# jacobwilliams/lbfgsb

Hardware: NVIDIA B200
Metric: lbfgsb_iterations_per_s (higher is better)
Workload: dtype f64

## Files before the change

### include/lbfgsb_b200.h

```cpp
#ifndef LBFGSB_B200_H
#define LBFGSB_B200_H

#include <stdint.h>

#ifdef __cplusplus
extern "C" {
#endif

#define LBFGSB_B200_MMAX 20

typedef struct lbfgsb_dev lbfgsb_dev_t;

int lbfgsb_b200_version(void);
const char* lbfgsb_b200_last_error(void);

void lbfgsb_setulb_f64(const int32_t* n, const int32_t* m, double* x, const double* l, const double* u,
                       const int32_t* nbd, double* f, double* g, const double* factr, const double* pgtol,
                       double* wa, int32_t* iwa, char* task, const int32_t* iprint, char* csave,
                       int32_t* lsave, int32_t* isave, double* dsave, const char* itfile, int32_t itfile_len);
void lbfgsb_setulb_f32(const int32_t* n, const int32_t* m, float* x, const float* l, const float* u,
                       const int32_t* nbd, float* f, float* g, const float* factr, const float* pgtol,
                       float* wa, int32_t* iwa, char* task, const int32_t* iprint, char* csave,
                       int32_t* lsave, int32_t* isave, float* dsave, const char* itfile, int32_t itfile_len);
void lbfgsb_host_release(int32_t* isave);
// ... 87 lines not shown

typedef struct lbfgsb_batch lbfgsb_batch_t;
lbfgsb_batch_t* lbfgsb_batch_create(int32_t nprob, int64_t n, int32_t m, int32_t real_kind, void* cuda_stream);
void lbfgsb_batch_destroy(lbfgsb_batch_t* h);
void lbfgsb_batch_setulb_dev_f64(lbfgsb_batch_t* h, double* x_dev, const double* l_dev, const double* u_dev, const int32_t* nbd_dev,
                                 double* f_dev, double* g_dev, const double* factr, const double* pgtol, char* task, char* csave,
                                 int32_t* lsave, int32_t* isave, double* dsave);
void lbfgsb_batch_setulb_dev_f32(lbfgsb_batch_t* h, float* x_dev, const float* l_dev, const float* u_dev, const int32_t* nbd_dev,
                                 float* f_dev, float* g_dev, const float* factr, const float* pgtol, char* task, char* csave,
                                 int32_t* lsave, int32_t* isave, float* dsave);
int lbfgsb_batch_counts(lbfgsb_batch_t* h, int32_t* n_fg, int32_t* n_newx, int32_t* n_done);
void* lbfgsb_batch_stream(lbfgsb_batch_t* h);
void* lbfgsb_batch_fg_mask(lbfgsb_batch_t* h);
int lbfgsb_batch_get_iwhere(lbfgsb_batch_t* h, int32_t* iwhere_host);
int lbfgsb_problem_rosenbrock_batch_f64(int32_t nprob, int64_t n, const double* x_dev, double* g_dev, double* f_dev,
                                        const int32_t* mask_dev, void* cuda_stream);
int lbfgsb_problem_rosenbrock_batch_f32(int32_t nprob, int64_t n, const float* x_dev, float* g_dev, float* f_dev,
                                        const int32_t* mask_dev, void* cuda_stream);

int lbfgsb_test_projgr_f64(int64_t n, const double* l, const double* u, const int32_t* nbd, const double* x,
                           const double* g, double* sbgnrm_out);
int lbfgsb_test_sum_f64(int64_t n, const double* a, const double* b, double* out);
int lbfgsb_test_sum_f32(int64_t n, const float* a, const float* b, float* out);
int lbfgsb_test_sort_f64(int64_t n, const double* t_dev, int32_t* order_out_dev, double* sorted_out_dev);
int lbfgsb_test_host_heap_group_f64(int64_t nb, const double* t_host, double tk, int32_t* group_out, int64_t* group_count);
int lbfgsb_test_heap_order_f64(int64_t n, const double* t_dev, int32_t* order_out_dev);
int lbfgsb_test_formk_delta_f64(int64_t n, int32_t m, int32_t col, int32_t head, int64_t ldw, const double* ws_dev,
                                const double* wy_dev, const unsigned char* state_dev, double* out_host);
int lbfgsb_test_formk_delta_f32(int64_t n, int32_t m, int32_t col, int32_t head, int64_t ldw, const float* ws_dev,
                                const float* wy_dev, const unsigned char* state_dev, float* out_host);
int lbfgsb_test_dense_f64(int32_t op, int32_t m, int32_t col, double theta, double* a, double* b, double* c,
                          int32_t* info);
int lbfgsb_test_dcsrch_f64(double f, double g, double* stp, double stpmax, int32_t* task, int32_t* isave2,
                           double* dsave13);

#ifdef __cplusplus
}
#endif
#endif
```

### lbfgsb_b200/csrc/common.cuh

```cuda
#pragma once
#include <cuda_runtime.h>
#include <stdint.h>
#include <float.h>
#include <math.h>

#include "../../include/lbfgsb_b200_shape.h"

typedef long long i64;

#define LB_MMAX 20
#define LB_KMAX (6 * LB_MMAX + 8)
#define LB_IMAX 8

enum {
    TK_START = 0, TK_FG_START = 1, TK_FG_LNSRCH = 2, TK_NEW_X = 3, TK_CONV_PG = 4, TK_CONV_F = 5,
    TK_ABNORMAL = 6, TK_RESTART = 7, TK_STOP = 8,
    TK_ERR_N = 10, TK_ERR_M = 11, TK_ERR_FACTR = 12, TK_ERR_NBD = 13, TK_ERR_INFEAS = 14
};
enum { PAUSE_NONE = 0, PAUSE_CLASSIFY = 1, PAUSE_WALK = 2, PAUSE_GCP_FREEV = 3, PAUSE_DELTA = 4, PAUSE_BACKTRACK = 5, PAUSE_LSINIT = 6 };
enum {
    CS_START = 0, CS_FG = 1, CS_CONV = 2, CS_WARN_ROUND = 3, CS_WARN_XTOL = 4, CS_WARN_STPMAX = 5,
    CS_WARN_STPMIN = 6, CS_ERR_STP_LT_MIN = 10, CS_ERR_STP_GT_MAX = 11, CS_ERR_G_GE_0 = 12,
    CS_ERR_FTOL = 13, CS_ERR_GTOL = 14, CS_ERR_XTOL = 15, CS_ERR_STPMIN = 16, CS_ERR_STPMAX = 17,
    CS_BLANK = 99
};
__host__ __device__ inline bool cs_is_warn(int c) { return c >= CS_WARN_ROUND && c <= CS_WARN_STPMIN; }
__host__ __device__ inline bool cs_is_err(int c) { return c >= CS_ERR_STP_LT_MIN && c <= CS_ERR_STPMAX; }
// ... 9 lines not shown
    EV_LNSRCH_RESTART = 8,
    EV_SKIP = 9,
    EV_FORMT_FAIL = 10
};
#define LB_EVMAX 24

template <typename T> struct Real;
template <> struct Real<double> {
    static constexpr int VEC = LBFGSB_VEC_F64;
    static constexpr int UNROLL = LBFGSB_UNROLL_F64;
    typedef double2 vec_t;
    typedef int2 ivec_t;
    typedef unsigned long long key_t;
    __host__ __device__ static double eps() { return DBL_EPSILON; }
};
template <> struct Real<float> {
    static constexpr int VEC = LBFGSB_VEC_F32;
    static constexpr int UNROLL = LBFGSB_UNROLL_F32;
    typedef float2 vec_t;
    typedef int2 ivec_t;
    typedef unsigned int key_t;
    __host__ __device__ static float eps() { return FLT_EPSILON; }
};

template <typename T>
struct DevState {
    int go;
    int pause;
    int in_body;
    int restart;
    int need_walk;
    int cauchy_mode;
    int do_subspace, do_formk, do_delta, do_backtrack, do_update, do_step, do_restore;
    int fuse_uc;
    int classify_done;
    int lsinit_done;
    int spec_step;
    int step_done;
    int do_unstep;
    int lazy_gcp;
    int fuse_gf;
    int lazy_z;
    int p2p_timeout;
    int z_in_x;
    int save_z;
    int task, csave, info;
// ... 706 lines not shown
```

### lbfgsb_b200/csrc/engine.cu

```cuda
#include <cuda_runtime.h>
#include <dlfcn.h>
#include <stdarg.h>
#include <stdio.h>
#include <stdlib.h>
#include <string.h>

#include <mutex>
#include <string>
#include <unordered_set>
#include <vector>

#include "../../include/lbfgsb_b200.h"
#include "cauchy_walk.cuh"
#include "kernels_tma.cuh"
#include "cauchy_walk_dist.cuh"
#include "batch.cuh"
#include "host_print.h"
#include <algorithm>

static thread_local std::string g_last_error;
static void set_error(const char* fmt, ...) {
    char buf[512];
    va_list ap;
    va_start(ap, fmt);
// ... 68 lines not shown
    __syncthreads();
    if (threadIdx.x == 0) *flag_host = seq;
}

__global__ void __launch_bounds__(256) k_publish_g(const unsigned* src, unsigned* dst_host, int words, volatile unsigned long long* flag_host,
                                                   unsigned long long* counter) {
    for (int q = threadIdx.x; q < words; q += blockDim.x) dst_host[q] = src[q];
    __threadfence_system();
    __syncthreads();
    if (threadIdx.x == 0) { const unsigned long long v = *counter + 1; *counter = v; *flag_host = v; }
}

struct EngineBase {
    virtual ~EngineBase() {}
    int real_kind;
    lbprint::Ctx pr;
};

template <typename T>
struct Engine : EngineBase {
    i64 n = 0, n_global = 0, offset = 0;
    int m = 0, mt = 0;
    bool fused = false;
    cudaStream_t stream = 0;
    bool own_stream = false;
    Wk<T> w;
    WalkBuf<T> wb;
    DevState<T>* s_dev = nullptr;
    DevState<T>* s_host = nullptr;
    size_t header_bytes = 0;
    int* tile_counts = nullptr; i64* tile_offsets = nullptr; i64 ntiles = 0;
    int* rs_counts = nullptr;
    SortCtl* ctl_el = nullptr;
    SortCtl* ctl_host = nullptr;
    T* tmpAB = nullptr; T* tmpF = nullptr; unsigned long long* jmin = nullptr;
    T* fd_parts = nullptr; T* delta = nullptr; T* delta_all = nullptr; T* delta_sum = nullptr;
    std::vector<void*> allocs;
    int R = 1, rank = 0;
    ncclComm_t comm = nullptr;
    Red<T>* rec_local = nullptr; Red<T>* rec_all = nullptr;
    unsigned long long* samp_local = nullptr; unsigned long long* samp_all = nullptr; unsigned long long* spl_dev = nullptr;
    DwCtl* dctl = nullptr; i64* pos_all = nullptr; SortCtl* ctl_d = nullptr;
    RoundRec* rr_local = nullptr; RoundRec* rr_all = nullptr;
    WalkCarry<T>* carry_local = nullptr; WalkCarry<T>* carry_all = nullptr;
    struct DynBuf { void* p = nullptr; size_t cap = 0; };
    DynBuf dw_send, dw_recv, dw_k0, dw_k1, dw_v0, dw_v1;
// ... 68 lines not shown
        p2p = true;
        for (int q = 0; q < R; ++q) p2p = p2p && oks[q];
        return true;
    }

    template <typename P> bool dalloc(P** p, size_t bytes) {
        void* q = nullptr;
        if (bytes == 0) bytes = 16;
        cudaError_t e = cudaMalloc(&q, bytes);
        if (e != cudaSuccess) { set_error("cudaMalloc(%zu) failed: %s", bytes, cudaGetErrorString(e)); return false; }
        allocs.push_back(q);
        *p = (P*)q;
        return true;
    }

    bool init(i64 n_, i64 off_, i64 ng_, int m_, cudaStream_t st, ncclComm_t cm, int rank_, int world_) {
        n = n_; offset = off_; n_global = ng_; m = m_; R = world_; rank = rank_; comm = cm;
        real_kind = (int)sizeof(T);
        mt = (m <= 5) ? 5 : (m <= 10 ? 10 : 20);
        fused = (mt == 5 ? fused_passes_ok<T, 5>() : (mt == 10 ? fused_passes_ok<T, 10>() : fused_passes_ok<T, 20>()));
        if (const char* e = getenv("LBFGSB_B200_NO_FUSION")) { if (e[0] == '1') fused = false; }
        fast = fused;
        if (const char* e = getenv("LBFGSB_B200_NO_FAST")) { if (e[0] == '1') fast = false; }
        if (const char* e = getenv("LBFGSB_B200_NO_TIMERS")) { if (e[0] == '1') timers = false; }
        if (const char* e = getenv("LBFGSB_B200_NO_SMALL_ROUNDS")) { if (e[0] == '1') { small_rounds = false; small_sort = false; } }
        if (const char* e = getenv("LBFGSB_B200_NO_BP_HINT")) { if (e[0] == '1') { bp_hint_ok = false; walk_gf_ok = false; } }
        if (!(mt == 5 ? set_smem_attrs<5>() : (mt == 10 ? set_smem_attrs<10>() : set_smem_attrs<20>()))) return false;
        for (int q = 0; q < F_COUNT; ++q) { fam_ms[q] = 0; fam_calls[q] = 0; }
        if (st) stream = st;
        else { CK(cudaStreamCreateWithFlags(&stream, cudaStreamNonBlocking)); own_stream = true; }
        memset(&w, 0, sizeof w);
        w.n = n; w.m = m; w.off = offset;
        w.ldw = (n + 31) / 32 * 32;
        const size_t vb = (size_t)w.ldw * sizeof(T);
        if (!dalloc(&w.ws, vb * m) || !dalloc(&w.wy, vb * m)) return false;
        if (!dalloc(&w.z, vb) || !dalloc(&w.r, vb) || !dalloc(&w.d, vb) || !dalloc(&w.t, vb) || !dalloc(&w.xp, vb) || !dalloc(&w.gold, vb)) return false;
        if (!dalloc(&w.iwhere, (size_t)w.ldw * 4) || !dalloc(&w.state, (size_t)w.ldw)) return false;
        if (!dalloc(&w.part, sizeof(T) * LB_KMAX * LBFGSB_GRID) || !dalloc(&w.ipart, sizeof(i64) * LB_IMAX * LBFGSB_GRID)) return false;
        if (!dalloc(&w.part2, sizeof(T) * LB_KMAX * LBFGSB_GRID) || !dalloc(&w.ipart2, sizeof(i64) * LB_IMAX * LBFGSB_GRID)) return false;
        if (!dalloc(&s_dev, sizeof(DevState<T>))) return false;
        CK(cudaMemsetAsync(s_dev, 0, sizeof(DevState<T>), stream));
        {
            i64 lim = (i64)1 << 28;
            if (R > 1) lim = (i64)1 << 26;
            if (const char* e = getenv("LBFGSB_B200_TIE_LIMIT")) lim = atoll(e);
            CK(cudaMemcpyAsync(&s_dev->tie_limit, &lim, sizeof lim, cudaMemcpyHostToDevice, stream));
        }
        CK(cudaMemsetAsync(w.ws, 0, vb * m, stream));
        CK(cudaMemsetAsync(w.wy, 0, vb * m, stream));
        w.s = s_dev;
        CK(cudaHostAlloc((void**)&s_host, sizeof(DevState<T>) + 64, cudaHostAllocMapped));
        memset(s_host, 0, sizeof(DevState<T>) + 64);
        pub_flag = (volatile unsigned long long*)((char*)s_host + ((sizeof(DevState<T>) + 7) / 8) * 8);
        if (const char* e = getenv("LBFGSB_B200_SYNC")) { if (e[0] == 'm') publish = false; }
        CK(cudaMallocHost((void**)&ctl_host, sizeof(SortCtl)));
// ... 152 lines not shown
        return true;
    }
#define LG LBFGSB_GRID, LBFGSB_BLOCK, 0, stream
#define LS 1, LB_SCALAR_THREADS, 0, stream
#define MTCALL(kern, smemfn, ...)                                                                          \
    do {                                                                                                   \
        if (mt == 5) kern<T, 5><<<LBFGSB_GRID, LB_TMA_THREADS, smemfn<T, 5>(), stream>>>(__VA_ARGS__);        \
        else if (mt == 10) kern<T, 10><<<LBFGSB_GRID, LB_TMA_THREADS, smemfn<T, 10>(), stream>>>(__VA_ARGS__); \
        else kern<T, 20><<<LBFGSB_GRID, LB_TMA_THREADS, smemfn<T, 20>(), stream>>>(__VA_ARGS__);              \
    } while (0)

    template <int MT> void launch_update_classify() {
        if constexpr (fused_passes_ok<T, MT>()) k_update_classify<T, MT><<<LBFGSB_GRID, LB_TMA_THREADS, smem_update_classify<T, MT>(), stream>>>(w);
    }
    template <int MT> void launch_formk_cmprlb() {
        if constexpr (fused_passes_ok<T, MT>()) k_formk_cmprlb<T, MT, 0><<<LBFGSB_GRID, LB_TMA_THREADS, smem_formk_cmprlb<T, MT>(), stream>>>(w);
    }
    template <int MT> void launch_formk_cmprlb_gf() {
        if constexpr (fused_passes_ok<T, MT>()) k_formk_cmprlb<T, MT, 1><<<LBFGSB_GRID, LB_TMA_THREADS, smem_formk_cmprlb<T, MT>(), stream>>>(w);
    }
    template <int MT> void launch_formk_cmprlb_gf2() {
        if constexpr (fused_passes_ok<T, MT>()) k_formk_cmprlb<T, MT, 2><<<LBFGSB_GRID, LB_TMA_THREADS, smem_formk_cmprlb<T, MT>(), stream>>>(w);
    }
    template <int MT> void launch_subsm_lsinit() {
        if constexpr (fused_passes_ok<T, MT>()) k_subsm_lsinit<T, MT, 0><<<LBFGSB_GRID, LB_TMA_THREADS, smem_subsm<T, MT>(), stream>>>(w);
    }
    template <int MT> void launch_subsm_dir() {
        if constexpr (fused_passes_ok<T, MT>()) k_subsm_lsinit<T, MT, 1><<<LBFGSB_GRID, LB_TMA_THREADS, smem_subsm<T, MT>(), stream>>>(w);
    }
#define MTFUSED(fn) do { if (mt == 5) fn<5>(); else if (mt == 10) fn<10>(); else fn<20>(); } while (0)

    template <int MT> bool set_smem_attrs() {
        CK(cudaFuncSetAttribute(k_update<T, MT>, cudaFuncAttributeMaxDynamicSharedMemorySize, (int)smem_update<T, MT>()));
        CK(cudaFuncSetAttribute(k_cauchy_classify<T, MT>, cudaFuncAttributeMaxDynamicSharedMemorySize, (int)smem_classify<T, MT>()));
        CK(cudaFuncSetAttribute(k_formk_gram<T, MT>, cudaFuncAttributeMaxDynamicSharedMemorySize, (int)smem_formk<T, MT>()));
        CK(cudaFuncSetAttribute(k_cmprlb_wv<T, MT>, cudaFuncAttributeMaxDynamicSharedMemorySize, (int)smem_cmprlb<T, MT>()));
        CK(cudaFuncSetAttribute(k_subsm_step<T, MT>, cudaFuncAttributeMaxDynamicSharedMemorySize, (int)smem_subsm<T, MT>()));
        if constexpr (fused_passes_ok<T, MT>()) {
            CK(cudaFuncSetAttribute(k_update_classify<T, MT>, cudaFuncAttributeMaxDynamicSharedMemorySize, (int)smem_update_classify<T, MT>()));
            CK(cudaFuncSetAttribute(k_formk_cmprlb<T, MT, 0>, cudaFuncAttributeMaxDynamicSharedMemorySize, (int)smem_formk_cmprlb<T, MT>()));
            CK(cudaFuncSetAttribute(k_formk_cmprlb<T, MT, 1>, cudaFuncAttributeMaxDynamicSharedMemorySize, (int)smem_formk_cmprlb<T, MT>()));
            CK(cudaFuncSetAttribute(k_formk_cmprlb<T, MT, 2>, cudaFuncAttributeMaxDynamicSharedMemorySize, (int)smem_formk_cmprlb<T, MT>()));
            CK(cudaFuncSetAttribute(k_subsm_lsinit<T, MT, 0>, cudaFuncAttributeMaxDynamicSharedMemorySize, (int)smem_subsm<T, MT>()));
            CK(cudaFuncSetAttribute(k_subsm_lsinit<T, MT, 1>, cudaFuncAttributeMaxDynamicSharedMemorySize, (int)smem_subsm<T, MT>()));
        }
        return true;
    }

    static unsigned long long key_of(T t) {
        typename Real<T>::key_t k;
        memcpy(&k, &t, sizeof k);
        return (unsigned long long)k;
    }
    int run_round(const BpRange& rg, bool first = false) {
        begin(F_WALK_COMPACT);
        if (first) k_bp_count<T, true><<<LG>>>(w, rg, tile_counts);
        else k_bp_count<T, false><<<LG>>>(w, rg, tile_counts);
        k_walk_round_local<T><<<1, 1024, 0, stream>>>(w, tile_counts, tile_offsets, ntiles, wb.ctl, rr_local);
        end(F_WALK_COMPACT, 2);
        if (R > 1 && !allgather(rr_local, rr_all, sizeof(RoundRec))) return -1;
        k_walk_round_begin<T><<<1, 32, 0, stream>>>(w, R > 1 ? rr_all : rr_local, R, n_global); launches++;
        if (!sync_state()) return -1;
        if (s_host->walk_closed) return 1;
        if (s_host->walk_rcount > 0) {
            begin(F_WALK_COMPACT); k_bp_write<T><<<LG>>>(w, rg, tile_counts, tile_offsets, wb.k0, wb.v0); end(F_WALK_COMPACT);
            begin(F_WALK_SORT); enqueue_sort(wb.k0, wb.k1, wb.v0, wb.v1, wb.ctl, s_host->walk_lcount); end(F_WALK_SORT, 0);
            if (R > 1) { if (!round_scan_sharded()) return -1; }
// ... 413 lines not shown
                    if (!site(site_freev())) return false;
                    begin(F_SCALAR); s_freev<T><<<LS>>>(w, dist(), n_global, 1); end(F_SCALAR);
                }
            }
            if (from <= PAUSE_DELTA) {
                if (from == PAUSE_DELTA) phase(PH_SUBSPACE);
                begin(F_FORMK_DELTA);
                k_el_count<T><<<LG>>>(w, tile_counts);
                k_tile_scan<T><<<1, 1024, 0, stream>>>(w, 1, tile_counts, tile_offsets, ntiles, ctl_el);
                k_flag_write<T, 1><<<LG>>>(w, tile_counts, tile_offsets, wb.k0, wb.v0);
                k_formk_delta<T><<<fd_grid<T>(), 256, 0, stream>>>(w, wb.v0, ctl_el, fd_parts);
                k_formk_delta_final<T><<<(6 * LB_MMAX * LB_MMAX + 255) / 256, 256, 0, stream>>>(w, fd_parts, fd_grid<T>(), delta);
                end(F_FORMK_DELTA, 5);
                if (!site(site_formk(mt))) return false;
                if (R > 1) {
                    if (p2p) { delta_seq++; k_delta_push<T><<<1, 256, 0, stream>>>(w, delta, peers_delta, peers, R, rank, delta_seq); launches++; }
                    else if (!allgather(delta, delta_all, sizeof(T) * 6 * LB_MMAX * LB_MMAX)) return false;
                }
                begin(F_SCALAR); s_formk_dense<T><<<LS>>>(w, dist(), mt, R > 1 ? delta_all : delta, delta_sum); end(F_SCALAR);
                if (!fused) { begin(F_CMPRLB_WV); MTCALL(k_cmprlb_wv, smem_cmprlb, w); end(F_CMPRLB_WV); }
                if (!site(site_wv(mt))) return false;
                begin(F_SCALAR); s_subsm_dense<T><<<LS>>>(w, dist(), mt, fused ? 1 : 0); end(F_SCALAR);
                if (fused) { begin(F_SUBSM_LSINIT); MTFUSED(launch_subsm_lsinit); end(F_SUBSM_LSINIT); }
                else { begin(F_SUBSM_STEP); MTCALL(k_subsm_step, smem_subsm, w); end(F_SUBSM_STEP); }
                if (!site(site_subsm())) return false;
                begin(F_SCALAR); s_subsm_post<T><<<LS>>>(w, dist(), fused ? 1 : 0); end(F_SCALAR);
            }
            if (from <= PAUSE_BACKTRACK) {
                if (from == PAUSE_BACKTRACK) phase(PH_SUBSPACE);
                begin(F_BACKTRACK);
                if (fused) { MTFUSED(launch_subsm_dir); launches++; }
                k_bt_alpha<T><<<LG>>>(w);
                if (!site(site_bt())) return false;
                s_bt<T><<<LS>>>(w, dist(), offset);
                k_bt_apply<T><<<LG>>>(w);
                end(F_BACKTRACK, 3);
            }
            phase(PH_LNSRCH);
            begin(F_LS_INIT); k_ls_init<T><<<LG>>>(w); end(F_LS_INIT);
            if (!site(site_lsinit())) return false;
            begin(F_SCALAR); s_ls_init<T><<<LS>>>(w, dist()); end(F_SCALAR);
            begin(F_LS_STEP); k_ls_step<T><<<LG>>>(w); end(F_LS_STEP);
            phase(PH_END);
            if (!sync_state()) return false;
            if (s_host->do_step) x_changed = true;
            if (!s_host->restart) break;
            begin(F_SCALAR); s_restart_body<T><<<1, 32, 0, stream>>>(w); end(F_SCALAR);
// ... 855 lines not shown
        T av[VEC], bv[VEC];
        ldv<T>(a, base, n, av); ldv<T>(b, base, n, bv);
#pragma unroll
        for (int v = 0; v < VEC; ++v) if (base + v < n) acc[0] = acc[0] + av[v] * bv[v];
    }
    block_sum_store<T, 1>(acc, 1, sm, part);
}
template <typename T>
__global__ void k_test_sum_final(const T* part, T* out) {
    T s = final_sum_warp<T>(part);
    if (threadIdx.x == 0) out[0] = s;
}
template <typename T>
static int test_sum_impl(i64 n, const T* a, const T* b, T* out) {
    T* part = nullptr;
    if (cudaMalloc(&part, sizeof(T) * (LBFGSB_GRID + 1)) != cudaSuccess) return 1;
    k_test_sum<T><<<LBFGSB_GRID, LBFGSB_BLOCK>>>(n, a, b, part);
    k_test_sum_final<T><<<1, 32>>>(part, part + LBFGSB_GRID);
    cudaError_t e = cudaMemcpy(out, part + LBFGSB_GRID, sizeof(T), cudaMemcpyDeviceToHost);
    cudaFree(part);
    return e != cudaSuccess;
}

__global__ void k_test_dense(int op, int m, int col, double theta, double* a, double* b, double* c, int* info, DevState<double>* st) {
    if (blockIdx.x != 0 || threadIdx.x >= 32) return;
    int r = 0;
    if (op >= 10 && op <= 14) {
        if (op == 10) r = wdense::dpofa<double>(a, m, col);
        else if (op == 11) r = wdense::dtrsl<double>(a, m, col, b, 1);
        else if (op == 12) r = wdense::dtrsl<double>(a, m, col, b, 11);
        else if (op == 13) r = wdense::bmv<double>(m, a, b, col, c, c + 2 * m);
        else r = wdense::formt<double>(m, c, a, b, col, theta);
        if (threadIdx.x == 0) *info = r;
        return;
    }
    if (op == 15) {
        if (threadIdx.x == 0) {
            st->m = m; st->col = col; st->theta = theta; st->do_formk = 1; st->updatd = 0; st->do_delta = 0; st->iupdat = m + 1;
            st->restart = 0; st->in_body = 1; st->ev_n = 0;
            for (int q = 0; q < m * m; ++q) st->sy[q] = b[q];
        }
        __syncwarp();
        Red<double>* red = nullptr;
        w_formk_dense<double>(st, *red, m <= 5 ? 5 : (m <= 10 ? 10 : 20), (const double*)nullptr, c, a);
        if (threadIdx.x == 0) *info = st->restart ? 1 : 0;
        return;
// ... 538 lines not shown
int lbfgsb_problem_quadratic_f32(int64_t n, const float* x, float* g, float* f_out, void* st, int64_t off, uint64_t seed,
                                 float xl, float xr, void* scratch) {
    return quadratic_impl<float>(n, x, g, f_out, st, off, seed, xl, xr, scratch);
}

int lbfgsb_test_projgr_f64(int64_t n, const double* l, const double* u, const int32_t* nbd, const double* x, const double* g,
                           double* out) {
    Wk<double> w; memset(&w, 0, sizeof w);
    DevState<double>* s = nullptr; double* part = nullptr;
    if (cudaMalloc(&s, sizeof(DevState<double>)) || cudaMalloc(&part, sizeof(double) * (LBFGSB_GRID + 1))) return 1;
    int one = 1;
    cudaMemcpy(&s->go, &one, sizeof(int), cudaMemcpyHostToDevice);
    w.n = n; w.l = l; w.u = u; w.nbd = nbd; w.x = (double*)x; w.g = (double*)g; w.part = part; w.s = s;
    k_projgr<double><<<LBFGSB_GRID, LBFGSB_BLOCK>>>(w);
    std::vector<double> hp(LBFGSB_GRID);
    cudaError_t e = cudaMemcpy(hp.data(), part, sizeof(double) * LBFGSB_GRID, cudaMemcpyDeviceToHost);
    double r = 0; for (double v : hp) r = v > r ? v : r;
    *out = r;
    cudaFree(s); cudaFree(part);
    return e != cudaSuccess;
}
int lbfgsb_test_sum_f64(int64_t n, const double* a, const double* b, double* out) { return test_sum_impl<double>(n, a, b, out); }
int lbfgsb_test_sum_f32(int64_t n, const float* a, const float* b, float* out) { return test_sum_impl<float>(n, a, b, out); }

int lbfgsb_test_sort_f64(int64_t n, const double* t, int32_t* order_out, double* sorted_out) {
    typedef unsigned long long K;
    K *k0, *k1; int *v0, *v1, *cnt; SortCtl* ctl;
    if (cudaMalloc(&k0, 8 * n) || cudaMalloc(&k1, 8 * n) || cudaMalloc(&v0, 4 * n) || cudaMalloc(&v1, 4 * n) ||
        cudaMalloc(&cnt, 4 * 256 * LB_RS_GRID) || cudaMalloc(&ctl, sizeof(SortCtl))) return 1;
    cudaMemcpy(k0, t, 8 * n, cudaMemcpyDeviceToDevice);
    k_test_iota<K><<<256, 256>>>(v0, n);
    k_test_setctl<<<1, 32>>>(ctl, n);
    for (int pass = 0; pass < 8; ++pass) {
        k_rs_hist<K><<<LB_RS_GRID, 256>>>(k0, k1, ctl, pass * 8, cnt);
        k_rs_scan<<<1, 1024>>>(cnt, ctl, LB_RS_GRID);
        k_rs_scatter<K><<<LB_RS_GRID, 256>>>(k0, k1, v0, v1, ctl, pass * 8, cnt);
        k_rs_flip<<<1, 32>>>(ctl);
    }
    SortCtl hc;
    cudaMemcpy(&hc, ctl, sizeof hc, cudaMemcpyDeviceToHost);
    cudaMemcpy(order_out, hc.cur ? v1 : v0, 4 * n, cudaMemcpyDeviceToDevice);
    cudaError_t e = cudaMemcpy(sorted_out, hc.cur ? k1 : k0, 8 * n, cudaMemcpyDeviceToDevice);
    cudaFree(k0); cudaFree(k1); cudaFree(v0); cudaFree(v1); cudaFree(cnt); cudaFree(ctl);
    return e != cudaSuccess || cudaGetLastError() != cudaSuccess;
}
int lbfgsb_test_host_heap_group_f64(int64_t nb, const double* t_host, double tk, int32_t* group_out, int64_t* group_count) {
// ... 135 lines not shown
```

### lbfgsb_b200/csrc/kernels_stream.cuh

```cuda
#pragma once
#include "common.cuh"

template <typename T>
struct Wk {
    i64 n, ldw;
    i64 off;
    int m;
    T *ws, *wy;
    T *z, *r, *d, *t, *xp;
    T* gold;
    int* iwhere;
    unsigned char* state;
    T* part;
    i64* ipart;
    T* part2;
    i64* ipart2;
    DevState<T>* s;
    T* x; const T* l; const T* u; const int* nbd; T* g;
    int bp_hint;
};

#define LB_SLOT(part, k) ((part) + (i64)(k) * LBFGSB_GRID)
#define LB_INF(T) ((T)INFINITY)
#define LB_I64MAX 0x7fffffffffffffffLL

template <typename T>
__global__ void __launch_bounds__(LBFGSB_BLOCK) k_errclb(Wk<T> w) {
    constexpr int VEC = Real<T>::VEC;
    i64 k6 = -1, k7 = -1;
    LB_FOR_TILES(T, w.n, base) {
        T l[VEC], u[VEC]; int nb[VEC];
        ldv<T>(w.l, base, w.n, l); ldv<T>(w.u, base, w.n, u); ldvi<T>(w.nbd, base, w.n, nb);
#pragma unroll
        for (int v = 0; v < VEC; ++v) {
            i64 i = base + v;
            if (i < w.n) {
                if (nb[v] < 0 || nb[v] > 3) k6 = i;
                if (nb[v] == 2 && l[v] > u[v]) k7 = i;
            }
        }
    }
    i64 m6 = k6, m7 = k7;
// ... 342 lines not shown
```

### lbfgsb_b200/csrc/kernels_tma.cuh

```cuda
#pragma once
#include "kernels_stream.cuh"
#include "tma_pipe.cuh"

template <typename T, int MT> struct SubT { static constexpr int v = (sizeof(T) * MT <= 80) ? 256 : 128; };

template <typename T> struct SpecializeFullHistory { static constexpr bool value = sizeof(T) == 4; };
template <bool B> struct BoolC { static constexpr bool value = B; };

#define LB_DYN_STAGES(dyn) (dyn)

template <typename T>
__device__ __forceinline__ void pipe_add_w(PipeSrc* ps, const Wk<T>& w, int head0, int count, unsigned slot) {
    int pj = head0;
    for (int j = 0; j < count; ++j) {
        pipe_add(ps, w.wy + (i64)pj * w.ldw, (int)sizeof(T), slot);
        pipe_add(ps, w.ws + (i64)pj * w.ldw, (int)sizeof(T), slot);
        pj = (pj + 1 == w.m) ? 0 : pj + 1;
    }
}

template <typename T, int MT>
__global__ void __launch_bounds__(LB_TMA_THREADS, 1) k_update(Wk<T> w) {
    constexpr int VEC = Real<T>::VEC;
    constexpr int SUBT = SubT<T, MT>::v;
// ... 291 lines not shown
                }
            }
        }
#pragma unroll
        for (int j = 0; j < MT; ++j) {
            if (j < col) {
                T wy[VEC], wsv[VEC];
                lds_real<T>(sb, OW + (2 * j) * G::REAL_SLOT, lt, wy);
                lds_real<T>(sb, OW + (2 * j + 1) * G::REAL_SLOT, lt, wsv);
#pragma unroll
                for (int v = 0; v < VEC; ++v)
                    if (fr[v]) {
                        acc[j] = acc[j] + wy[v] * r[v];
                        acc[MT + j] = acc[MT + j] + wsv[v] * r[v];
                    }
            }
        }
        stv<T>(w.r, base, n, r);
    });
    block_sum_store<T, 2 * MT>(acc, 2 * MT, sm, w.part2);
}
template <typename T, int MT> constexpr unsigned smem_cmprlb() { return pipe_smem_bytes<T, SubT<T, MT>::v>(3 + 2 * MT, 0, 1); }

template <typename T, int MT>
__global__ void __launch_bounds__(LB_TMA_THREADS, 1) k_subsm_step(Wk<T> w) {
    constexpr int VEC = Real<T>::VEC;
    constexpr int SUBT = SubT<T, MT>::v;
    typedef PipeGeom<T, SUBT> G;
    extern __shared__ __align__(128) char dyn[];
    __shared__ unsigned long long full[2 * LB_PIPE_STAGES];
    __shared__ PipeSrc ps;
    __shared__ T sm[LBFGSB_BLOCK / 32];
    __shared__ i64 smi[LBFGSB_BLOCK / 32];
    const DevState<T>* s = w.s;
    if (!s->go || !s->in_body || !s->do_subspace) return;
    const i64 n = w.n;
    const int col = s->col, head0 = s->head - 1;
    const T theta = s->theta, rtheta = (T)1 / theta;
    constexpr unsigned OZ = 0, OX = G::REAL_SLOT, OG = 2 * G::REAL_SLOT, OR = 3 * G::REAL_SLOT, OL = 4 * G::REAL_SLOT,
                       OU = 5 * G::REAL_SLOT, OW = 6 * G::REAL_SLOT;
    if (threadIdx.x == 0) {
        pipe_begin(&ps);
        pipe_add(&ps, w.z, sizeof(T), G::REAL_SLOT);
        pipe_add(&ps, w.x, sizeof(T), G::REAL_SLOT);
        pipe_add(&ps, w.g, sizeof(T), G::REAL_SLOT);
        pipe_add(&ps, w.r, sizeof(T), G::REAL_SLOT);
        pipe_add(&ps, w.l, sizeof(T), G::REAL_SLOT);
        pipe_add(&ps, w.u, sizeof(T), G::REAL_SLOT);
        pipe_add_w<T>(&ps, w, head0, col, G::REAL_SLOT);
        pipe_add(&ps, w.nbd, 4, G::INT_SLOT);
        pipe_add(&ps, w.state, 1, G::BYTE_SLOT);
        pipe_end(&ps);
    }
    const unsigned onb = OW + 2u * (unsigned)col * G::REAL_SLOT, ost = onb + G::INT_SLOT;
    T wv1[MT], wv2[MT];
#pragma unroll
    for (int j = 0; j < MT; ++j) { wv1[j] = (j < col) ? s->wv[j] : (T)0; wv2[j] = (j < col) ? s->wv[col + j] : (T)0; }
    T acc[1]; acc[0] = (T)0;
    i64 iwd = 0;
    tma_pass<T, SUBT>(n, &ps, LB_DYN_STAGES(dyn), full, [&](i64 base, const char* sb, int lt) {
        int st[VEC];
        lds_byte<T>(sb, ost, lt, st);
        bool fr[VEC]; bool any = false;
#pragma unroll
        for (int v = 0; v < VEC; ++v) { fr[v] = (base + v < n) && (st[v] & 1); any |= fr[v]; }
        T z[VEC], x[VEC], g[VEC];
        lds_real<T>(sb, OZ, lt, z); lds_real<T>(sb, OX, lt, x); lds_real<T>(sb, OG, lt, g);
        stv<T>(w.xp, base, n, z);
        if (any) {
            T dk[VEC], l[VEC], u[VEC]; int nb[VEC];
            lds_real<T>(sb, OR, lt, dk); lds_real<T>(sb, OL, lt, l); lds_real<T>(sb, OU, lt, u);
            lds_int<T>(sb, onb, lt, nb);
#pragma unroll
            for (int j = 0; j < MT; ++j) {
                if (j < col) {
                    T wy[VEC], wsv[VEC];
                    lds_real<T>(sb, OW + (2 * j) * G::REAL_SLOT, lt, wy);
                    lds_real<T>(sb, OW + (2 * j + 1) * G::REAL_SLOT, lt, wsv);
#pragma unroll
                    for (int v = 0; v < VEC; ++v) dk[v] = dk[v] + wy[v] * wv1[j] / theta + wsv[v] * wv2[j];
                }
            }
#pragma unroll
            for (int v = 0; v < VEC; ++v) {
                dk[v] = rtheta * dk[v];
                if (fr[v]) {
                    T xk = z[v];
                    if (nb[v] != 0) {
                        if (nb[v] == 1) { z[v] = dense::tmax(l[v], xk + dk[v]); if (z[v] == l[v]) iwd = 1; }
                        else if (nb[v] == 2) {
                            xk = dense::tmax(l[v], xk + dk[v]);
                            z[v] = dense::tmin(u[v], xk);
                            if (z[v] == l[v] || z[v] == u[v]) iwd = 1;
                        } else if (nb[v] == 3) { z[v] = dense::tmin(u[v], xk + dk[v]); if (z[v] == u[v]) iwd = 1; }
                    } else z[v] = xk + dk[v];
                }
            }
            stv<T>(w.r, base, n, dk);
            stv<T>(w.z, base, n, z);
        }
#pragma unroll
        for (int v = 0; v < VEC; ++v)
            if (base + v < n) acc[0] = acc[0] + (z[v] - x[v]) * g[v];
    });
    block_sum_store<T, 1>(acc, 1, sm, w.part);
// ... 247 lines not shown
#pragma unroll
            for (int j = 0; j < MT; ++j) {
                if (j < col) {
                    T wy[VEC], wsv[VEC];
                    if (PREF) {
#pragma unroll
                        for (int v = 0; v < VEC; ++v) { wy[v] = wyn[v]; wsv[v] = wsn[v]; }
                        if (j + 1 < MT) {
                            lds_real_v<T>(sb, OW + (2 * j + 2) * G::REAL_SLOT, lt, wyn);
                            lds_real_v<T>(sb, OW + (2 * j + 3) * G::REAL_SLOT, lt, wsn);
                        }
                    } else {
                        lds_real<T>(sb, OW + (2 * j) * G::REAL_SLOT, lt, wy);
                        lds_real<T>(sb, OW + (2 * j + 1) * G::REAL_SLOT, lt, wsv);
                    }
#pragma unroll
                    for (int v = 0; v < VEC; ++v) {
                        const T py = wy[v] * r[v], psv = wsv[v] * r[v];
                        if (fr[v]) { aw[j] = aw[j] + py; aw[MT + j] = aw[MT + j] + psv; }
                    }
                }
            }
        }
        stv<T>(w.r, base, n, r);
    });
    };
    pass(BoolC<false>{});
    if (gram) block_sum_store<T, 4 * MT>(af, 4 * MT, sm, w.part);
    block_sum_store<T, 2 * MT>(aw, 2 * MT, sm, w.part2);
    if (gf) {
        i64 r0 = block_isum((i64)nfr, smi), r1 = block_isum((i64)nen, smi), r2 = block_isum((i64)nle, smi);
        if (threadIdx.x == 0) {
            LB_SLOT(w.ipart, 0)[blockIdx.x] = r0; LB_SLOT(w.ipart, 1)[blockIdx.x] = r1;
            LB_SLOT(w.ipart, 2)[blockIdx.x] = r2;
        }
    }
}
template <typename T, int MT> constexpr unsigned smem_formk_cmprlb() { return pipe_smem_bytes<T, SubT<T, MT>::v>(3 + 2 * MT, 1, 1); }

template <typename T, int MT, int PASS>
__global__ void __launch_bounds__(LB_TMA_THREADS, 1) k_subsm_lsinit(Wk<T> w) {
    constexpr int VEC = Real<T>::VEC;
    constexpr int SUBT = SubT<T, MT>::v;
    typedef PipeGeom<T, SUBT> G;
    extern __shared__ __align__(128) char dyn[];
    __shared__ unsigned long long full[2 * LB_PIPE_STAGES];
    __shared__ PipeSrc ps;
    __shared__ T sm[2 * (LBFGSB_BLOCK / 32)];
    __shared__ T smm[LBFGSB_BLOCK / 32];
    __shared__ i64 smi[LBFGSB_BLOCK / 32];
    const DevState<T>* s = w.s;
    if (!s->go || s->pause || !s->in_body || !s->do_subspace) return;
    const bool spec = s->spec_step != 0;
    if (PASS == 1 && !(spec && s->do_backtrack)) return;
    const i64 n = w.n;
    const int col = s->col, head0 = s->head - 1;
    const T theta = s->theta, rtheta = (T)1 / theta;
    const bool bounds = (s->cnstnd && s->iter != 0);
    const bool lz = s->lazy_z != 0;
    const T tsum = s->tsum;
    const bool axpy = tsum != (T)0;
    constexpr unsigned OX = 0, OG = G::REAL_SLOT, OL = 2 * G::REAL_SLOT, OU = 3 * G::REAL_SLOT, OR = 4 * G::REAL_SLOT,
                       OZ = 5 * G::REAL_SLOT;
    const unsigned OW = (lz ? 5u : 6u) * G::REAL_SLOT;
    if (threadIdx.x == 0) {
        pipe_begin(&ps);
        pipe_add(&ps, PASS == 1 ? w.t : w.x, sizeof(T), G::REAL_SLOT);
        pipe_add(&ps, w.g, sizeof(T), G::REAL_SLOT);
        pipe_add(&ps, w.l, sizeof(T), G::REAL_SLOT);
        pipe_add(&ps, w.u, sizeof(T), G::REAL_SLOT);
        pipe_add(&ps, w.r, sizeof(T), G::REAL_SLOT);
        if (!lz) pipe_add(&ps, w.z, sizeof(T), G::REAL_SLOT);
        pipe_add_w<T>(&ps, w, head0, col, G::REAL_SLOT);
        pipe_add(&ps, w.nbd, 4, G::INT_SLOT);
        pipe_add(&ps, w.state, 1, G::BYTE_SLOT);
        pipe_end(&ps);
    }
    T wv1[MT], wv2[MT];
#pragma unroll
    for (int j = 0; j < MT; ++j) { wv1[j] = (j < col) ? s->wv[j] : (T)0; wv2[j] = (j < col) ? s->wv[col + j] : (T)0; }
    T acc[2]; acc[0] = (T)0; acc[1] = (T)0;
    T smx = LB_INF(T);
    i64 iwd = 0;
    auto pass = [&](auto full_c) {
    constexpr bool FULLC = decltype(full_c)::value;
    const unsigned onb = OW + 2u * (unsigned)(FULLC ? MT : col) * G::REAL_SLOT, ost = onb + G::INT_SLOT;
    tma_pass<T, SUBT>(n, &ps, LB_DYN_STAGES(dyn), full, [&](i64 base, const char* sb, int lt) {
        int st[VEC];
        lds_byte<T>(sb, ost, lt, st);
        bool fr[VEC]; bool any = false;
#pragma unroll
        for (int v = 0; v < VEC; ++v) { fr[v] = (base + v < n) && (st[v] & 1); any |= fr[v]; }
        if (PASS == 1 && !any && !lz) return;
        T z[VEC], x[VEC], g[VEC];
        lds_real<T>(sb, OX, lt, x); lds_real<T>(sb, OG, lt, g);
        if (lz) {
#pragma unroll
            for (int v = 0; v < VEC; ++v) z[v] = axpy ? (x[v] + tsum * ((st[v] & 4) ? -g[v] : (T)0)) : x[v];
        } else lds_real<T>(sb, OZ, lt, z);
        T dk[VEC];
        if (any) {
            lds_real<T>(sb, OR, lt, dk);
#pragma unroll
            for (int j = 0; j < MT; ++j) {
                if (FULLC || j < col) {
                    T wy[VEC], wsv[VEC];
                    lds_real<T>(sb, OW + (2 * j) * G::REAL_SLOT, lt, wy);
                    lds_real<T>(sb, OW + (2 * j + 1) * G::REAL_SLOT, lt, wsv);
#pragma unroll
                    for (int v = 0; v < VEC; ++v) dk[v] = dk[v] + wy[v] * wv1[j] / theta + wsv[v] * wv2[j];
                }
            }
#pragma unroll
            for (int v = 0; v < VEC; ++v) dk[v] = rtheta * dk[v];
        }
        if (PASS == 1) {
            if (any) stv<T>(w.r, base, n, dk);
            if (lz) stv<T>(w.z, base, n, z);
            return;
        }
        T l[VEC], u[VEC]; int nb[VEC];
        lds_real<T>(sb, OL, lt, l); lds_real<T>(sb, OU, lt, u);
        lds_int<T>(sb, onb, lt, nb);
        if (!spec) stv<T>(w.xp, base, n, z);
        if (any) {
#pragma unroll
            for (int v = 0; v < VEC; ++v) {
                if (fr[v]) {
                    T xk = z[v];
                    if (nb[v] != 0) {
                        if (nb[v] == 1) { z[v] = dense::tmax(l[v], xk + dk[v]); if (z[v] == l[v]) iwd = 1; }
                        else if (nb[v] == 2) {
                            xk = dense::tmax(l[v], xk + dk[v]);
                            z[v] = dense::tmin(u[v], xk);
                            if (z[v] == l[v] || z[v] == u[v]) iwd = 1;
// ... 48 lines not shown
```

Baseline: 93.58.

## Recompute reduced gradient in subspace kernel and replace divisions with reciprocal refinement

The subspace-minimization kernels no longer load the stored r vector when z is lazily formed. They rebuild r from -theta*(z-x)-g plus a W·a correction, and the formk/cmprlb pass skips writing r. Per-element division by theta is replaced with a reciprocal multiply plus two FMA Newton refinement steps. An exponent range check falls back to true division whenever the result might not match exactly. This cuts streamed bytes and expensive f64 divides, at the cost of extra FMAs, a possible second pass, and more template variants; a classic env-var path is kept.

```diff
diff --git a/include/lbfgsb_b200.h b/include/lbfgsb_b200.h
--- a/include/lbfgsb_b200.h
+++ b/include/lbfgsb_b200.h
@@ -133,6 +133,8 @@
                            const double* g, double* sbgnrm_out);
 int lbfgsb_test_sum_f64(int64_t n, const double* a, const double* b, double* out);
 int lbfgsb_test_sum_f32(int64_t n, const float* a, const float* b, float* out);
+int lbfgsb_test_div_f64(int32_t on_device, int64_t n, const double* a, const double* b, double* q, double* ref);
+int lbfgsb_test_div_f32(int32_t on_device, int64_t n, const float* a, const float* b, float* q, float* ref);
 int lbfgsb_test_sort_f64(int64_t n, const double* t_dev, int32_t* order_out_dev, double* sorted_out_dev);
 int lbfgsb_test_host_heap_group_f64(int64_t nb, const double* t_host, double tk, int32_t* group_out, int64_t* group_count);
 int lbfgsb_test_heap_order_f64(int64_t n, const double* t_dev, int32_t* order_out_dev);
diff --git a/lbfgsb_b200/csrc/common.cuh b/lbfgsb_b200/csrc/common.cuh
--- a/lbfgsb_b200/csrc/common.cuh
+++ b/lbfgsb_b200/csrc/common.cuh
@@ -3,6 +3,7 @@
 #include <stdint.h>
 #include <float.h>
 #include <math.h>
+#include <string.h>
 
 #include "../../include/lbfgsb_b200_shape.h"
 
@@ -58,6 +59,52 @@
     typedef unsigned int key_t;
     __host__ __device__ static float eps() { return FLT_EPSILON; }
 };
+
+template <typename T> struct DivRange;
+template <> struct DivRange<double> {
+    static constexpr unsigned MASK = 0x7ff00000u, ONE = 0x00100000u, BIAS = 1023u, LIM = 896u;
+    __host__ __device__ static __forceinline__ unsigned hi(double v) {
+#ifdef __CUDA_ARCH__
+        return (unsigned)__double2hiint(v);
+#else
+        unsigned long long b; memcpy(&b, &v, sizeof b); return (unsigned)(b >> 32);
+#endif
+    }
+    __host__ __device__ static __forceinline__ double fma_(double a, double b, double c) { return fma(a, b, c); }
+};
+template <> struct DivRange<float> {
+    static constexpr unsigned MASK = 0x7f800000u, ONE = 0x00800000u, BIAS = 127u, LIM = 96u;
+    __host__ __device__ static __forceinline__ unsigned hi(float v) {
+#ifdef __CUDA_ARCH__
+        return __float_as_uint(v);
+#else
+        unsigned b; memcpy(&b, &v, sizeof b); return b;
+#endif
+    }
+    __host__ __device__ static __forceinline__ float fma_(float a, float b, float c) { return fmaf(a, b, c); }
+};
+template <typename T>
+__host__ __device__ __forceinline__ bool div_in_range(T v) {
+    typedef DivRange<T> D;
+    return (D::hi(v) & D::MASK) - (D::BIAS - D::LIM) * D::ONE <= 2u * D::LIM * D::ONE;
+}
+template <typename T>
+__host__ __device__ __forceinline__ T div_by_recip_try(T a, T b, T y, bool& exact) {
+    typedef DivRange<T> D;
+    const T q0 = a * y;
+    const T r0 = D::fma_(-b, q0, a);
+    const T q1 = D::fma_(r0, y, q0);
+    const T r1 = D::fma_(-b, q1, a);
+    const T q2 = D::fma_(r1, y, q1);
+    exact = exact & ((a == (T)0) | (div_in_range(a) & div_in_range(q0)));
+    return (a == (T)0) ? q0 : q2;
+}
+template <typename T>
+__host__ __device__ __forceinline__ T div_by_recip(T a, T b, T y) {
+    bool exact = div_in_range(b);
+    const T q = div_by_recip_try<T>(a, b, y, exact);
+    return exact ? q : a / b;
+}
 
 template <typename T>
 struct DevState {
diff --git a/lbfgsb_b200/csrc/engine.cu b/lbfgsb_b200/csrc/engine.cu
--- a/lbfgsb_b200/csrc/engine.cu
+++ b/lbfgsb_b200/csrc/engine.cu
@@ -114,6 +114,7 @@
     i64 n = 0, n_global = 0, offset = 0;
     int m = 0, mt = 0;
     bool fused = false;
+    bool subsm_classic = false;
     cudaStream_t stream = 0;
     bool own_stream = false;
     Wk<T> w;
@@ -228,6 +229,7 @@
         if (const char* e = getenv("LBFGSB_B200_NO_FUSION")) { if (e[0] == '1') fused = false; }
         fast = fused;
         if (const char* e = getenv("LBFGSB_B200_NO_FAST")) { if (e[0] == '1') fast = false; }
+        if (const char* e = getenv("LBFGSB_B200_SUBSM_CLASSIC")) { if (e[0] == '1') subsm_classic = true; }
         if (const char* e = getenv("LBFGSB_B200_NO_TIMERS")) { if (e[0] == '1') timers = false; }
         if (const char* e = getenv("LBFGSB_B200_NO_SMALL_ROUNDS")) { if (e[0] == '1') { small_rounds = false; small_sort = false; } }
         if (const char* e = getenv("LBFGSB_B200_NO_BP_HINT")) { if (e[0] == '1') { bp_hint_ok = false; walk_gf_ok = false; } }
@@ -237,6 +239,7 @@
         else { CK(cudaStreamCreateWithFlags(&stream, cudaStreamNonBlocking)); own_stream = true; }
         memset(&w, 0, sizeof w);
         w.n = n; w.m = m; w.off = offset;
+        w.reform_r = subsm_classic ? 0 : 1;
         w.ldw = (n + 31) / 32 * 32;
         const size_t vb = (size_t)w.ldw * sizeof(T);
         if (!dalloc(&w.ws, vb * m) || !dalloc(&w.wy, vb * m)) return false;
@@ -435,11 +438,17 @@
     template <int MT> void launch_formk_cmprlb_gf2() {
         if constexpr (fused_passes_ok<T, MT>()) k_formk_cmprlb<T, MT, 2><<<LBFGSB_GRID, LB_TMA_THREADS, smem_formk_cmprlb<T, MT>(), stream>>>(w);
     }
-    template <int MT> void launch_subsm_lsinit() {
-        if constexpr (fused_passes_ok<T, MT>()) k_subsm_lsinit<T, MT, 0><<<LBFGSB_GRID, LB_TMA_THREADS, smem_subsm<T, MT>(), stream>>>(w);
-    }
-    template <int MT> void launch_subsm_dir() {
-        if constexpr (fused_passes_ok<T, MT>()) k_subsm_lsinit<T, MT, 1><<<LBFGSB_GRID, LB_TMA_THREADS, smem_subsm<T, MT>(), stream>>>(w);
+    template <int MT, int PASS> void launch_subsm_pass() {
+        if constexpr (fused_passes_ok<T, MT>()) {
+            if (subsm_classic) k_subsm_lsinit<T, MT, PASS, true><<<LBFGSB_GRID, LB_TMA_THREADS, smem_subsm<T, MT>(), stream>>>(w);
+            else k_subsm_lsinit<T, MT, PASS, false><<<LBFGSB_GRID, LB_TMA_THREADS, smem_subsm<T, MT>(), stream>>>(w);
+        }
+    }
+    template <int MT> void launch_subsm_lsinit() { launch_subsm_pass<MT, 0>(); }
+    template <int MT> void launch_subsm_dir() { launch_subsm_pass<MT, 1>(); }
+    template <int MT> void launch_subsm_step() {
+        if (subsm_classic) k_subsm_step<T, MT, true><<<LBFGSB_GRID, LB_TMA_THREADS, smem_subsm<T, MT>(), stream>>>(w);
+        else k_subsm_step<T, MT, false><<<LBFGSB_GRID, LB_TMA_THREADS, smem_subsm<T, MT>(), stream>>>(w);
     }
 #define MTFUSED(fn) do { if (mt == 5) fn<5>(); else if (mt == 10) fn<10>(); else fn<20>(); } while (0)
 
@@ -448,14 +457,17 @@
         CK(cudaFuncSetAttribute(k_cauchy_classify<T, MT>, cudaFuncAttributeMaxDynamicSharedMemorySize, (int)smem_classify<T, MT>()));
         CK(cudaFuncSetAttribute(k_formk_gram<T, MT>, cudaFuncAttributeMaxDynamicSharedMemorySize, (int)smem_formk<T, MT>()));
         CK(cudaFuncSetAttribute(k_cmprlb_wv<T, MT>, cudaFuncAttributeMaxDynamicSharedMemorySize, (int)smem_cmprlb<T, MT>()));
-        CK(cudaFuncSetAttribute(k_subsm_step<T, MT>, cudaFuncAttributeMaxDynamicSharedMemorySize, (int)smem_subsm<T, MT>()));
+        CK(cudaFuncSetAttribute(k_subsm_step<T, MT, false>, cudaFuncAttributeMaxDynamicSharedMemorySize, (int)smem_subsm<T, MT>()));
+        CK(cudaFuncSetAttribute(k_subsm_step<T, MT, true>, cudaFuncAttributeMaxDynamicSharedMemorySize, (int)smem_subsm<T, MT>()));
         if constexpr (fused_passes_ok<T, MT>()) {
             CK(cudaFuncSetAttribute(k_update_classify<T, MT>, cudaFuncAttributeMaxDynamicSharedMemorySize, (int)smem_update_classify<T, MT>()));
             CK(cudaFuncSetAttribute(k_formk_cmprlb<T, MT, 0>, cudaFuncAttributeMaxDynamicSharedMemorySize, (int)smem_formk_cmprlb<T, MT>()));
             CK(cudaFuncSetAttribute(k_formk_cmprlb<T, MT, 1>, cudaFuncAttributeMaxDynamicSharedMemorySize, (int)smem_formk_cmprlb<T, MT>()));
             CK(cudaFuncSetAttribute(k_formk_cmprlb<T, MT, 2>, cudaFuncAttributeMaxDynamicSharedMemorySize, (int)smem_formk_cmprlb<T, MT>()));
-            CK(cudaFuncSetAttribute(k_subsm_lsinit<T, MT, 0>, cudaFuncAttributeMaxDynamicSharedMemorySize, (int)smem_subsm<T, MT>()));
-            CK(cudaFuncSetAttribute(k_subsm_lsinit<T, MT, 1>, cudaFuncAttributeMaxDynamicSharedMemorySize, (int)smem_subsm<T, MT>()));
+            CK(cudaFuncSetAttribute(k_subsm_lsinit<T, MT, 0, false>, cudaFuncAttributeMaxDynamicSharedMemorySize, (int)smem_subsm<T, MT>()));
+            CK(cudaFuncSetAttribute(k_subsm_lsinit<T, MT, 1, false>, cudaFuncAttributeMaxDynamicSharedMemorySize, (int)smem_subsm<T, MT>()));
+            CK(cudaFuncSetAttribute(k_subsm_lsinit<T, MT, 0, true>, cudaFuncAttributeMaxDynamicSharedMemorySize, (int)smem_subsm<T, MT>()));
+            CK(cudaFuncSetAttribute(k_subsm_lsinit<T, MT, 1, true>, cudaFuncAttributeMaxDynamicSharedMemorySize, (int)smem_subsm<T, MT>()));
         }
         return true;
     }
@@ -915,7 +927,7 @@
                 if (!site(site_wv(mt))) return false;
                 begin(F_SCALAR); s_subsm_dense<T><<<LS>>>(w, dist(), mt, fused ? 1 : 0); end(F_SCALAR);
                 if (fused) { begin(F_SUBSM_LSINIT); MTFUSED(launch_subsm_lsinit); end(F_SUBSM_LSINIT); }
-                else { begin(F_SUBSM_STEP); MTCALL(k_subsm_step, smem_subsm, w); end(F_SUBSM_STEP); }
+                else { begin(F_SUBSM_STEP); MTFUSED(launch_subsm_step); end(F_SUBSM_STEP); }
                 if (!site(site_subsm())) return false;
                 begin(F_SCALAR); s_subsm_post<T><<<LS>>>(w, dist(), fused ? 1 : 0); end(F_SCALAR);
             }
@@ -1817,6 +1829,24 @@
     return e != cudaSuccess;
 }
 
+template <typename T>
+__global__ void k_test_div(i64 n, const T* a, const T* b, T* q, T* ref) {
+    for (i64 i = blockIdx.x * (i64)blockDim.x + threadIdx.x; i < n; i += (i64)gridDim.x * blockDim.x) {
+        const T bi = b[i];
+        q[i] = div_by_recip<T>(a[i], bi, (T)1 / bi);
+        ref[i] = a[i] / bi;
+    }
+}
+template <typename T>
+static int test_div_impl(int on_device, i64 n, const T* a, const T* b, T* q, T* ref) {
+    if (!on_device) {
+        for (i64 i = 0; i < n; ++i) { q[i] = div_by_recip<T>(a[i], b[i], (T)1 / b[i]); ref[i] = a[i] / b[i]; }
+        return 0;
+    }
+    k_test_div<T><<<4 * 148, 256>>>(n, a, b, q, ref);
+    return cudaDeviceSynchronize() != cudaSuccess;
+}
+
 __global__ void k_test_dense(int op, int m, int col, double theta, double* a, double* b, double* c, int* info, DevState<double>* st) {
     if (blockIdx.x != 0 || threadIdx.x >= 32) return;
     int r = 0;
@@ -2401,6 +2431,12 @@
 }
 int lbfgsb_test_sum_f64(int64_t n, const double* a, const double* b, double* out) { return test_sum_impl<double>(n, a, b, out); }
 int lbfgsb_test_sum_f32(int64_t n, const float* a, const float* b, float* out) { return test_sum_impl<float>(n, a, b, out); }
+int lbfgsb_test_div_f64(int32_t on_device, int64_t n, const double* a, const double* b, double* q, double* ref) {
+    return test_div_impl<double>(on_device, n, a, b, q, ref);
+}
+int lbfgsb_test_div_f32(int32_t on_device, int64_t n, const float* a, const float* b, float* q, float* ref) {
+    return test_div_impl<float>(on_device, n, a, b, q, ref);
+}
 
 int lbfgsb_test_sort_f64(int64_t n, const double* t, int32_t* order_out, double* sorted_out) {
     typedef unsigned long long K;
diff --git a/lbfgsb_b200/csrc/kernels_stream.cuh b/lbfgsb_b200/csrc/kernels_stream.cuh
--- a/lbfgsb_b200/csrc/kernels_stream.cuh
+++ b/lbfgsb_b200/csrc/kernels_stream.cuh
@@ -18,6 +18,7 @@
     DevState<T>* s;
     T* x; const T* l; const T* u; const int* nbd; T* g;
     int bp_hint;
+    int reform_r;
 };
 
 #define LB_SLOT(part, k) ((part) + (i64)(k) * LBFGSB_GRID)
diff --git a/lbfgsb_b200/csrc/kernels_tma.cuh b/lbfgsb_b200/csrc/kernels_tma.cuh
--- a/lbfgsb_b200/csrc/kernels_tma.cuh
+++ b/lbfgsb_b200/csrc/kernels_tma.cuh
@@ -337,7 +337,36 @@
 }
 template <typename T, int MT> constexpr unsigned smem_cmprlb() { return pipe_smem_bytes<T, SubT<T, MT>::v>(3 + 2 * MT, 0, 1); }
 
-template <typename T, int MT>
+template <typename T, int MT, bool CLASSIC, typename G>
+__device__ __forceinline__ void subsm_dk(const char* sb, int lt, const T (&r)[Real<T>::VEC], unsigned OW, int ncol,
+                                         const T (&wv1)[MT], const T (&wv2)[MT], T theta, T rtheta, bool theta_ok,
+                                         T (&dk)[Real<T>::VEC]) {
+    constexpr int VEC = Real<T>::VEC;
+    auto chain = [&](auto recip_c) {
+        constexpr bool RECIP = decltype(recip_c)::value;
+        bool exact = true;
+#pragma unroll
+        for (int v = 0; v < VEC; ++v) dk[v] = r[v];
+#pragma unroll
+        for (int j = 0; j < MT; ++j) {
+            if (j < ncol) {
+                T wy[VEC], wsv[VEC];
+                lds_real<T>(sb, OW + (2 * j) * G::REAL_SLOT, lt, wy);
+                lds_real<T>(sb, OW + (2 * j + 1) * G::REAL_SLOT, lt, wsv);
+#pragma unroll
+                for (int v = 0; v < VEC; ++v) {
+                    const T a = wy[v] * wv1[j];
+                    const T q = RECIP ? div_by_recip_try<T>(a, theta, rtheta, exact) : a / theta;
+                    dk[v] = dk[v] + q + wsv[v] * wv2[j];
+                }
+            }
+        }
+        return exact;
+    };
+    if (CLASSIC || !theta_ok || !chain(BoolC<true>{})) chain(BoolC<false>{});
+}
+
+template <typename T, int MT, bool CLASSIC>
 __global__ void __launch_bounds__(LB_TMA_THREADS, 1) k_subsm_step(Wk<T> w) {
     constexpr int VEC = Real<T>::VEC;
     constexpr int SUBT = SubT<T, MT>::v;
@@ -352,6 +381,7 @@
     const i64 n = w.n;
     const int col = s->col, head0 = s->head - 1;
     const T theta = s->theta, rtheta = (T)1 / theta;
+    const bool theta_ok = div_in_range(theta);
     constexpr unsigned OZ = 0, OX = G::REAL_SLOT, OG = 2 * G::REAL_SLOT, OR = 3 * G::REAL_SLOT, OL = 4 * G::REAL_SLOT,
                        OU = 5 * G::REAL_SLOT, OW = 6 * G::REAL_SLOT;
     if (threadIdx.x == 0) {
@@ -384,18 +414,11 @@
         stv<T>(w.xp, base, n, z);
         if (any) {
             T dk[VEC], l[VEC], u[VEC]; int nb[VEC];
-            lds_real<T>(sb, OR, lt, dk); lds_real<T>(sb, OL, lt, l); lds_real<T>(sb, OU, lt, u);
+            T r[VEC];
+            lds_real<T>(sb, OR, lt, r);
+            subsm_dk<T, MT, CLASSIC, G>(sb, lt, r, OW, col, wv1, wv2, theta, rtheta, theta_ok, dk);
+            lds_real<T>(sb, OL, lt, l); lds_real<T>(sb, OU, lt, u);
             lds_int<T>(sb, onb, lt, nb);
-#pragma unroll
-            for (int j = 0; j < MT; ++j) {
-                if (j < col) {
-                    T wy[VEC], wsv[VEC];
-                    lds_real<T>(sb, OW + (2 * j) * G::REAL_SLOT, lt, wy);
-                    lds_real<T>(sb, OW + (2 * j + 1) * G::REAL_SLOT, lt, wsv);
-#pragma unroll
-                    for (int v = 0; v < VEC; ++v) dk[v] = dk[v] + wy[v] * wv1[j] / theta + wsv[v] * wv2[j];
-                }
-            }
 #pragma unroll
             for (int v = 0; v < VEC; ++v) {
                 dk[v] = rtheta * dk[v];
@@ -689,7 +712,7 @@
                 }
             }
         }
-        stv<T>(w.r, base, n, r);
+        if (GF != 1 || !w.reform_r) stv<T>(w.r, base, n, r);
     });
     };
     pass(BoolC<false>{});
@@ -705,7 +728,7 @@
 }
 template <typename T, int MT> constexpr unsigned smem_formk_cmprlb() { return pipe_smem_bytes<T, SubT<T, MT>::v>(3 + 2 * MT, 1, 1); }
 
-template <typename T, int MT, int PASS>
+template <typename T, int MT, int PASS, bool CLASSIC>
 __global__ void __launch_bounds__(LB_TMA_THREADS, 1) k_subsm_lsinit(Wk<T> w) {
     constexpr int VEC = Real<T>::VEC;
     constexpr int SUBT = SubT<T, MT>::v;
@@ -716,6 +739,7 @@
     __shared__ T sm[2 * (LBFGSB_BLOCK / 32)];
     __shared__ T smm[LBFGSB_BLOCK / 32];
     __shared__ i64 smi[LBFGSB_BLOCK / 32];
+    __shared__ T coef[2 * MT];
     const DevState<T>* s = w.s;
     if (!s->go || s->pause || !s->in_body || !s->do_subspace) return;
     const bool spec = s->spec_step != 0;
@@ -723,20 +747,23 @@
     const i64 n = w.n;
     const int col = s->col, head0 = s->head - 1;
     const T theta = s->theta, rtheta = (T)1 / theta;
+    const bool theta_ok = div_in_range(theta);
     const bool bounds = (s->cnstnd && s->iter != 0);
     const bool lz = s->lazy_z != 0;
     const T tsum = s->tsum;
     const bool axpy = tsum != (T)0;
+    const bool reform = lz && w.reform_r;
+    const bool uc = (!s->cnstnd && col > 0);
     constexpr unsigned OX = 0, OG = G::REAL_SLOT, OL = 2 * G::REAL_SLOT, OU = 3 * G::REAL_SLOT, OR = 4 * G::REAL_SLOT,
                        OZ = 5 * G::REAL_SLOT;
-    const unsigned OW = (lz ? 5u : 6u) * G::REAL_SLOT;
+    const unsigned OW = (4u + (reform ? 0u : 1u) + (lz ? 0u : 1u)) * G::REAL_SLOT;
     if (threadIdx.x == 0) {
         pipe_begin(&ps);
         pipe_add(&ps, PASS == 1 ? w.t : w.x, sizeof(T), G::REAL_SLOT);
         pipe_add(&ps, w.g, sizeof(T), G::REAL_SLOT);
         pipe_add(&ps, w.l, sizeof(T), G::REAL_SLOT);
         pipe_add(&ps, w.u, sizeof(T), G::REAL_SLOT);
-        pipe_add(&ps, w.r, sizeof(T), G::REAL_SLOT);
+        if (!reform) pipe_add(&ps, w.r, sizeof(T), G::REAL_SLOT);
         if (!lz) pipe_add(&ps, w.z, sizeof(T), G::REAL_SLOT);
         pipe_add_w<T>(&ps, w, head0, col, G::REAL_SLOT);
         pipe_add(&ps, w.nbd, 4, G::INT_SLOT);
@@ -746,6 +773,10 @@
     T wv1[MT], wv2[MT];
 #pragma unroll
     for (int j = 0; j < MT; ++j) { wv1[j] = (j < col) ? s->wv[j] : (T)0; wv2[j] = (j < col) ? s->wv[col + j] : (T)0; }
+    if (threadIdx.x < 2 * MT) {
+        const int j = threadIdx.x % MT;
+        coef[threadIdx.x] = (j < col) ? ((threadIdx.x < MT) ? s->a[j] : theta * s->a[col + j]) : (T)0;
+    }
     T acc[2]; acc[0] = (T)0; acc[1] = (T)0;
     T smx = LB_INF(T);
     i64 iwd = 0;
@@ -767,17 +798,25 @@
         } else lds_real<T>(sb, OZ, lt, z);
         T dk[VEC];
         if (any) {
-            lds_real<T>(sb, OR, lt, dk);
-#pragma unroll
-            for (int j = 0; j < MT; ++j) {
-                if (FULLC || j < col) {
-                    T wy[VEC], wsv[VEC];
-                    lds_real<T>(sb, OW + (2 * j) * G::REAL_SLOT, lt, wy);
-                    lds_real<T>(sb, OW + (2 * j + 1) * G::REAL_SLOT, lt, wsv);
-#pragma unroll
-                    for (int v = 0; v < VEC; ++v) dk[v] = dk[v] + wy[v] * wv1[j] / theta + wsv[v] * wv2[j];
-                }
-            }
+            T r[VEC];
+            if (reform) {
+#pragma unroll
+                for (int v = 0; v < VEC; ++v) r[v] = uc ? -g[v] : (-theta * (z[v] - x[v]) - g[v]);
+                if (!uc) {
+#pragma unroll
+                    for (int j = 0; j < MT; ++j) {
+                        if (FULLC || j < col) {
+                            T wy[VEC], wsv[VEC];
+                            lds_real<T>(sb, OW + (2 * j) * G::REAL_SLOT, lt, wy);
+                            lds_real<T>(sb, OW + (2 * j + 1) * G::REAL_SLOT, lt, wsv);
+                            const T a1 = coef[j], a2 = coef[MT + j];
+#pragma unroll
+                            for (int v = 0; v < VEC; ++v) r[v] = r[v] + wy[v] * a1 + wsv[v] * a2;
+                        }
+                    }
+                }
+            } else lds_real<T>(sb, OR, lt, r);
+            subsm_dk<T, MT, CLASSIC, G>(sb, lt, r, OW, FULLC ? MT : col, wv1, wv2, theta, rtheta, theta_ok, dk);
 #pragma unroll
             for (int v = 0; v < VEC; ++v) dk[v] = rtheta * dk[v];
         }
```

After: 95.43, median of 6. 1.02x the previous value.
